# edmundhung/SparkFM

Measured on AMD Instinct MI355X. Metric: nnz_per_sec_fm_sgd_training, higher is better.
Workload: dtype f32

## Files before the change

### sparkfm_amd/csrc/fm_forward.hip

```cpp
#include "fm_device.h"

#ifndef FMHIP_FWD_LDS_SHARE
#define FMHIP_FWD_LDS_SHARE 1
#endif
#ifndef FMHIP_FWD_AHEAD
#define FMHIP_FWD_AHEAD 1
#endif
#ifndef FMHIP_FWD_W_SPLIT
#define FMHIP_FWD_W_SPLIT 1
#endif
#ifndef FMHIP_EXP_NO_STREAM
#define FMHIP_EXP_NO_STREAM 0
#endif
#ifndef FMHIP_EXP_NO_MATH
#define FMHIP_EXP_NO_MATH 0
#endif
#ifndef FMHIP_EXP_NO_W
#define FMHIP_EXP_NO_W 0
#endif
#ifndef FMHIP_EXP_NO_GATHER
#define FMHIP_EXP_NO_GATHER 0
#endif
#ifndef FMHIP_EXP_L1_GATHER
#define FMHIP_EXP_L1_GATHER 0
// ... 5 lines not shown
#define FMHIP_EXP_PHASE_PROBE 0
#endif
#define FMHIP_FWD_ABLATIONS ((FMHIP_EXP_NO_STREAM ? 1 : 0) | (FMHIP_EXP_NO_MATH ? 2 : 0) | (FMHIP_EXP_NO_W ? 4 : 0) | (FMHIP_EXP_NO_GATHER ? 8 : 0) | \
                             (FMHIP_EXP_L1_GATHER ? 16 : 0) | (FMHIP_EXP_NO_HOT ? 32 : 0) | (FMHIP_EXP_PHASE_PROBE ? 64 : 0))
#if FMHIP_FWD_ABLATIONS && !defined(FMHIP_ABLATION_BUILD)
#error "a result-changing FMHIP_EXP_* ablation is set without FMHIP_ABLATION_BUILD: timing-only variants are built by tools/build_variant.sh"
#endif

namespace fmhip {
int forward_ablations() { return FMHIP_FWD_ABLATIONS; }
}

namespace fmhip {

std::atomic<int> g_tune[kTuneCount] = {60, 1, 0, 0, 2, 1, 0, 1, 0, 1, 0, 1, 4};

int padded_factors(int k) {
    int kp = 32;
    while (kp < k) kp <<= 1;
    return kp;
}

int forward_wt_occupancy(int Kp);

int forward_blocks_wt(int Kp, int64_t n_rows, int occ_cap) {
    const int64_t need = forward_blocks(Kp, n_rows);
    int occ = forward_wt_occupancy(Kp);
    if (occ_cap > 0 && occ_cap < occ) occ = occ_cap;
    const int64_t cap = (int64_t)256 * occ;
    return (int)(need < cap ? need : cap);
// ... 159 lines not shown
                if (MASKED) {
                    float4 tv = f4mul(t[j][jj], __int_as_float(xi[j]));
                    if (!live) tv = f4zero();
                    f4add(q[jj], tv);
                    f4sqacc(s[jj], tv);
                } else if (FMHIP_EXP_NO_MATH) {
                    q[jj].x += t[j][jj].x * __int_as_float(xi[j]);
                } else {
                    acc_entry(q[jj], s[jj], t[j][jj], __int_as_float(xi[j]));
                }
            }
        }
    }
}

template <int LPN, int J, int MODE, bool PACKED>
__device__ __forceinline__ void row_finish(const FwdArgs &a, int r, int l, float4 (&q)[J], float4 (&s)[J], float lin, float w0,
                                           float &st1, float &st2, float &stbad, float &stl) {
    constexpr int KP = 4 * LPN * J;
    const int kl = PACKED ? (a.pack_k >> 2) & (LPN - 1) : 0, kj = PACKED ? (a.pack_k >> 2) / LPN : 0, kc = a.pack_k & 3;
    if (fwd_mode(MODE) == kFwdPartA) {
        float sp = 0.f, lp = lin;
#pragma unroll
        for (int jj = 0; jj < J; ++jj) {
            float4 sj = s[jj];
            if (PACKED && jj == kj && l == kl) f4set(sj, kc, 0.f);
            sp += (sj.x + sj.y) + (sj.z + sj.w);
        }
#pragma unroll
        for (int m = LPN >> 1; m >= 1; m >>= 1) { sp += __shfl_xor(sp, m, LPN); lp += __shfl_xor(lp, m, LPN); }
        float4 *pr = reinterpret_cast<float4 *>(a.P + (size_t)r * KP) + l;
#pragma unroll
        for (int jj = 0; jj < J; ++jj) pr[jj * LPN] = q[jj];
        if (l == 0) { a.part_sl[2 * (size_t)r] = sp; a.part_sl[2 * (size_t)r + 1] = lp; }
// ... 9 lines not shown
                if (l == kl) { f4set(q[jj], kc, 0.f); f4set(s[jj], kc, 0.f); }
            }
        lin_all = a.sw * __shfl(lk, kl, LPN);
    }
    float u = 0.f;
#pragma unroll
    for (int jj = 0; jj < J; ++jj) u += f4sqminus(q[jj], s[jj]);
    float tot = fmaf(0.5f * a.sv * a.sv, u, a.sw * lin);
    if (fwd_mode(MODE) == kFwdPartB && l == 0) tot += fmaf(-0.5f * a.sv * a.sv, a.part_sl[2 * (size_t)r], a.sw * a.part_sl[2 * (size_t)r + 1]);
#pragma unroll
    for (int m = LPN >> 1; m >= 1; m >>= 1) tot += __shfl_xor(tot, m, LPN);
    const float yhat = w0 + (tot + lin_all);
    constexpr bool logistic = (MODE & kFwdLogistic) != 0;
    float e, lrow = 0.f;
    if constexpr (logistic) {
        const bool t = a.y[a.row0 + r] > 0.f;
        const float z = expf(-fabsf(yhat)), inv = 1.f / (1.f + z);
        const bool pos = yhat >= 0.f;
        e = t ? -(pos ? z * inv : inv) : (pos ? inv : z * inv);
        if constexpr (fwd_mode(MODE) == kFwdResidual) lrow = fmaxf(t ? -yhat : yhat, 0.f) + log1pf(z);
    } else {
        e = yhat - a.y[a.row0 + r];
    }
    if (fwd_mode(MODE) == kFwdTrain || fwd_mode(MODE) == kFwdPartB) {
        float4 *pr = reinterpret_cast<float4 *>(a.P + (size_t)r * KP) + l;
        const float es = e * a.sv;
#pragma unroll
        for (int jj = 0; jj < J; ++jj) {
            float4 o = f4mul(q[jj], es);
            if (PACKED && jj == kj && l == kl) f4set(o, kc, e);
            if (!PACKED && kEInP && jj == 0 && l < 8) o = embed_bits4(o, __float_as_uint(e) >> (4 * l));
            p_store(pr + jj * LPN, o);
        }
    } else if (fwd_mode(MODE) == kFwdQ) {
        float4 *pr = reinterpret_cast<float4 *>(a.P + (size_t)r * KP) + l;
#pragma unroll
        for (int jj = 0; jj < J; ++jj) pr[jj * LPN] = f4mul(q[jj], a.sv);
// ... 48 lines not shown
    float *wt = lds + (size_t)T * KP;
    {
        const float4 *src = reinterpret_cast<const float4 *>(a.V);
        float4 *dst = reinterpret_cast<float4 *>(vt);
        const int n4 = T * (KP / 4);
        for (int i = threadIdx.x; i < n4; i += kLdsBlock) dst[i] = src[i];
        for (int i = threadIdx.x; i < T; i += kLdsBlock) wt[i] = a.w[i];
    }
    __syncthreads();
    const int l = threadIdx.x & (LPN - 1);
    const int slot = threadIdx.x / LPN;
    const float w0 = *a.w0;
    const __amdgpu_buffer_rsrc_t vr = make_rsrc(a.V, a.v_bytes);
    float st1 = 0.f, st2 = 0.f, stbad = 0.f, stl = 0.f;
    for (int ri = blockIdx.x * SLOTS + slot; ri < a.n_rows; ri += gridDim.x * SLOTS) {
        const int r = a.order ? a.order[ri] : ri;
        const int64_t p0 = a.row_ptr[a.row0 + r], p1 = a.row_ptr[a.row0 + r + 1];
        float4 q[J], s[J];
#pragma unroll
        for (int jj = 0; jj < J; ++jj) { q[jj] = f4zero(); s[jj] = f4zero(); }
        float lin = 0.f;
        for (int64_t base = p0; base < p1; base += LPN) {
            const int64_t p = base + l;
            int c = -1;
            float x = 0.f;
            if (p < p1) {
                c = stream_load(a.col + p);
                x = stream_load(a.val + p);
                const float wv = c < T ? wt[c] : a.w[c];
                lin = fmaf(wv, x, lin);
            }
#pragma unroll
// ... 14 lines not shown
                        tl[j][jj] = lp[jj * LPN];
                    }
                }
#pragma unroll
                for (int j = 0; j < CH; ++j) {
#pragma unroll
                    for (int jj = 0; jj < J; ++jj) {
                        const float4 t = hot[j] ? tl[j][jj] : tg[j][jj];
                        const float4 tv = f4mul(t, xs[j]);
                        f4add(q[jj], tv);
                        f4sqacc(s[jj], tv);
                    }
                }
            }
        }
        row_finish<LPN, J, MODE, false>(a, r, l, q, s, lin, w0, st1, st2, stbad, stl);
    }
    block_stats<kLdsBlock, MODE == (kFwdResidual | kFwdLogistic)>(a.bsum, st1, st2, stbad, stl);
}

template <bool WT, bool BUF>
__device__ __forceinline__ float w_lookup(const FwdArgs &a, __amdgpu_buffer_rsrc_t wr, const float *wt, int T, int c) {
    if (BUF && FMHIP_FWD_W_SPLIT) {
        const bool in_tile = WT && (uint32_t)c < (uint32_t)T;
        const float wg = buf_load1(wr, in_tile ? kOob : (uint32_t)c * 4u);
        if (!WT) return wg;
        const float wl = wt[in_tile ? c : 0];
        return in_tile ? wl : wg;
    }
    const int cc = c < 0 ? 0 : c;
    const float v = (WT && cc < T) ? wt[cc] : a.w[cc];
// ... 12 lines not shown
    const int T = WT ? a.wt_rows : 0;
    const __amdgpu_buffer_rsrc_t vr = make_rsrc(a.V, a.v_bytes);
    const __amdgpu_buffer_rsrc_t wr = make_rsrc(a.w, a.v_bytes / KPW);
    const int32_t *colb = a.col + a.nz0;
    const float *valb = a.val + a.nz0;
    float st1 = 0.f, st2 = 0.f, stbad = 0.f, stl = 0.f;
    if (BUF && FMHIP_FWD_AHEAD) {
#if FMHIP_EXP_PHASE_PROBE
        {
            const bool late = FMHIP_EXP_PHASE_PROBE >= 1000 ? (((blockIdx.x >> 3) ^ (blockIdx.x >> 8)) & 1) != 0 : __builtin_amdgcn_readfirstlane((int)(threadIdx.x >> 6)) >= 2;
            if (late)
                for (int i = 0; i < FMHIP_EXP_PHASE_PROBE % 1000; ++i) __builtin_amdgcn_s_sleep(1);
        }
#endif
        for (int ri = blockIdx.x * SLOTS + slot; ri < a.n_rows; ri += gridDim.x * SLOTS) {
            const int r = a.order ? a.order[ri] : ri;
            float4 xh = f4zero();
            if (HOT) xh = hot_load(a, r, l);
            const uint32_t p0 = (uint32_t)((fwd_mode(MODE) == kFwdPartB ? a.row_split[a.row0 + r] : a.row_ptr[a.row0 + r]) - a.nz0),
                           p1 = (uint32_t)((fwd_mode(MODE) == kFwdPartA ? a.row_split[a.row0 + r] : a.row_ptr[a.row0 + r + 1]) - a.nz0);
            float4 q[J], s[J];
#pragma unroll
            for (int jj = 0; jj < J; ++jj) {
                q[jj] = fwd_mode(MODE) == kFwdPartB ? reinterpret_cast<const float4 *>(a.P + (size_t)r * KPW)[jj * LPN + l] : f4zero();
                s[jj] = f4zero();
            }
            float lin = 0.f;
            if (HOT && !FMHIP_EXP_NO_HOT) {
                if (hot_plain) hot_prologue<LPN, J, !PACKED, false>(xh, vh, wh, l, q, s, lin);
                else hot_prologue<LPN, J, !PACKED, true>(xh, vh, wh, l, q, s, lin);
            }
            int c_n = -1;
            float x_n = 0.f;
            bool live_n = p0 + l < p1;
            if (live_n) { c_n = stream_load(colb + (p0 + l)); x_n = stream_load(valb + (p0 + l)); }
// ... 8 lines not shown
                    typedef __attribute__((address_space(1))) const float gflt;
                    gint *cp = (gint *)(live_n ? colb + pos : reinterpret_cast<const int32_t *>(a.w0));
                    gflt *xp = (gflt *)(live_n ? valb + pos : a.w0);
                    asm volatile("" : "+v"(cp), "+v"(xp));
                    c_n = *cp;
                    x_n = *xp;
                } else {
                    live_n = true; c_n = -1; x_n = 0.f;
                    if (pos < p1) { c_n = stream_load(colb + pos); x_n = stream_load(valb + pos); }
                }
                float wv = 0.f;
                if (!PACKED && !FMHIP_EXP_NO_W && c >= 0) wv = w_lookup<WT, BUF>(a, wr, wt, T, c);
                fwd_step<LPN, J, CH, false, BUF, PH == 1>(a.V, vr, slot_publish<LPN>(stage, c, x, l), c, x, LPN, l, q, s);
                if (!PACKED) lin = fmaf(wv, x, lin);
            }
            row_finish<LPN, J, MODE, PACKED>(a, r, l, q, s, lin, w0, st1, st2, stbad, stl);
        }
        block_stats<kBlock, MODE == (kFwdResidual | kFwdLogistic)>(a.bsum, st1, st2, stbad, stl);
        return;
    }
    for (int ri = blockIdx.x * SLOTS + slot; ri < a.n_rows; ri += gridDim.x * SLOTS) {
        const int r = a.order ? a.order[ri] : ri;
        float4 xh = f4zero();
        if (HOT) xh = hot_load(a, r, l);
        const uint32_t p0 = (uint32_t)((fwd_mode(MODE) == kFwdPartB ? a.row_split[a.row0 + r] : a.row_ptr[a.row0 + r]) - a.nz0),
                       p1 = (uint32_t)((fwd_mode(MODE) == kFwdPartA ? a.row_split[a.row0 + r] : a.row_ptr[a.row0 + r + 1]) - a.nz0);
        float4 q[J], s[J];
#pragma unroll
        for (int jj = 0; jj < J; ++jj) {
            q[jj] = fwd_mode(MODE) == kFwdPartB ? reinterpret_cast<const float4 *>(a.P + (size_t)r * KPW)[jj * LPN + l] : f4zero();
            s[jj] = f4zero();
        }
        float lin = 0.f;
        if (HOT && !FMHIP_EXP_NO_HOT) {
            if (hot_plain) hot_prologue<LPN, J, !PACKED, false>(xh, vh, wh, l, q, s, lin);
            else hot_prologue<LPN, J, !PACKED, true>(xh, vh, wh, l, q, s, lin);
        }
        uint32_t base = p0;
        for (; base + LPN <= p1; base += LPN) {
            const int c = FMHIP_EXP_NO_STREAM ? (int)((base + l) & 1023u) : stream_load(colb + (base + l));
            const float x = FMHIP_EXP_NO_STREAM ? 1.f : stream_load(valb + (base + l));
// ... 2 lines not shown
            fwd_step<LPN, J, CH, false, BUF>(a.V, vr, slot_publish<LPN>(stage, c, x, l), c, x, LPN, l, q, s);
            if (!PACKED) lin = fmaf(wv, x, lin);
        }
        if (base < p1) {
            const uint32_t p = base + l;
            int c = BUF ? -1 : 0;
            float x = 0.f, wv = 0.f;
            if (p < p1) {
                c = stream_load(colb + p);
                x = stream_load(valb + p);
                if (!PACKED && !FMHIP_EXP_NO_W) wv = w_lookup<WT, BUF>(a, wr, wt, T, c);
            }
            fwd_step<LPN, J, CH, !BUF, BUF>(a.V, vr, slot_publish<LPN>(stage, c, x, l), c, x, (int)(p1 - base), l, q, s);
            if (!PACKED) lin = fmaf(wv, x, lin);
        }
        row_finish<LPN, J, MODE, PACKED>(a, r, l, q, s, lin, w0, st1, st2, stbad, stl);
    }
    block_stats<kBlock, MODE == (kFwdResidual | kFwdLogistic)>(a.bsum, st1, st2, stbad, stl);
}

#ifndef FMHIP_FWD_PLAIN_WGS
#define FMHIP_FWD_PLAIN_WGS 5
#endif
template <int LPN, int J, int MODE, bool PACKED, bool HOT, bool BUF>
__global__ __launch_bounds__(kBlock, (LPN * J <= 8 && HOT ? FMHIP_FWD_PLAIN_WGS : 1)) void k_forward(FwdArgs a) {
    constexpr int KP = 4 * LPN * J;
    __shared__ __attribute__((aligned(16))) float vh[HOT ? kHotT * KP : 4];
    __shared__ float wh[HOT ? kHotT : 1];
    bool hot_plain = false;
    if (HOT) hot_plain = hot_stage<KP>(a, vh, wh);
    forward_rows<LPN, J, MODE, PACKED, HOT, false, BUF>(a, nullptr, vh, wh, hot_plain);
// ... 14 lines not shown
    else __syncthreads();
    forward_rows<LPN, J, MODE, false, HOT, true, BUF, PH>(a, wt, vh, wh, hot_plain);
}

template <int LPN, int J, int MODE, bool PACKED>
__global__ __launch_bounds__(kBlock) void k_forward_pass_b(FwdArgs a) {
    constexpr int KP = 4 * LPN * J;
    constexpr int SLOTS = kBlock / LPN;
    const int l = threadIdx.x & (LPN - 1);
    const int slot = threadIdx.x / LPN;
    const float w0 = *a.w0;
    const int32_t *colb = a.col + a.nz0;
    const float *valb = a.val + a.nz0;
    float st1 = 0.f, st2 = 0.f, stbad = 0.f, stl = 0.f;
    for (int ri = blockIdx.x * SLOTS + slot; ri < a.n_rows; ri += gridDim.x * SLOTS) {
        const int r = a.order ? a.order[ri] : ri;
        const uint32_t p0 = (uint32_t)(a.row_split[a.row0 + r] - a.nz0), p1 = (uint32_t)(a.row_ptr[a.row0 + r + 1] - a.nz0);
        float4 q[J], s[J];
#pragma unroll
        for (int jj = 0; jj < J; ++jj) {
            q[jj] = reinterpret_cast<const float4 *>(a.P + (size_t)r * KP)[jj * LPN + l];
            s[jj] = f4zero();
        }
        float lin = 0.f;
        for (uint32_t p = p0; p < p1; ++p) {
            const int c = colb[p];
            const float x = valb[p];
            const float4 *vp = reinterpret_cast<const float4 *>(a.V + (size_t)(uint32_t)c * KP) + l;
#pragma unroll
            for (int jj = 0; jj < J; ++jj) acc_entry(q[jj], s[jj], vp[jj * LPN], x);
            if (!PACKED && l == 0) lin = fmaf(a.w[c], x, lin);
        }
        row_finish<LPN, J, MODE, PACKED>(a, r, l, q, s, lin, w0, st1, st2, stbad, stl);
    }
    block_stats<kBlock, false>(a.bsum, st1, st2, stbad, stl);
}

__global__ __launch_bounds__(kBlock) void k_reduce_blocks(const double *bsum, int32_t nblocks, int32_t n_rows, float *scal,
                                                         double *acc) {
    __shared__ double sh[3][kBlock / 64];
    reduce_blocks_body(bsum, nblocks, n_rows, scal, acc, sh);
}

__global__ __launch_bounds__(kBlock) void k_reduce_blocks_logloss(const double *bsum, int32_t nblocks, int32_t n_rows, float *scal,
                                                                 double *acc) {
    __shared__ double sh[4][kBlock / 64];
    reduce_blocks_body<true>(bsum, nblocks, n_rows, scal, acc, sh);
}
// ... 80 lines not shown
hipError_t fwd_launch_pass(const FwdArgs &a0, hipStream_t s, int *n_partials) {
    if constexpr (LPN * J > 16) {
        return hipErrorInvalidValue;
    } else {
        FwdArgs a = a0;
        const bool hot_here = a.hot_T && (fwd_mode(MODE) == kFwdPartB) == (a.hot_in_b != 0);
        if (!hot_here) a.hot_T = 0;
        if (fwd_mode(MODE) == kFwdPartB) a.variant = 0;
        if (a.variant == 20) a.variant = a.hot_T ? 60 : 0;
        const FwdPlan pl = fwd_plan<LPN, J>(a);
        if (n_partials) *n_partials = pl.blocks;
        const dim3 g((unsigned)pl.blocks), b(kBlock);
        const bool buf = a.v_bytes != 0;
        if constexpr (fwd_mode(MODE) == kFwdPartB) {
            if (!a.hot_T) {
                a.order = nullptr;
                if (a.pack_k >= 0) hipLaunchKernelGGL((k_forward_pass_b<LPN, J, MODE, true>), g, b, 0, s, a);
                else hipLaunchKernelGGL((k_forward_pass_b<LPN, J, MODE, false>), g, b, 0, s, a);
                return hipGetLastError();
            }
        }
        if constexpr (fwd_mode(MODE) == kFwdPartA) {
            if (pl.var == 60) {
                const size_t lds_bytes = (size_t)a.wt_rows * sizeof(float);
                if (a.hot_T) {
                    if (buf) launch_wt<LPN, J, MODE, true, true>(a, g, b, lds_bytes, s);
                    else launch_wt<LPN, J, MODE, true, false>(a, g, b, lds_bytes, s);
                } else {
                    if (buf) launch_wt<LPN, J, MODE, false, true>(a, g, b, lds_bytes, s);
                    else launch_wt<LPN, J, MODE, false, false>(a, g, b, lds_bytes, s);
                }
// ... 110 lines not shown
```

### sparkfm_amd/csrc/fm_kernels.h

```cpp
#pragma once
#include <hip/hip_runtime.h>
#include <stdint.h>

#include <atomic>

#include "fm_constants.h"

namespace fmhip {

constexpr int kPartPad = 4;
constexpr int kScalars = 8;
constexpr int kGradHead = 32;

enum { kTuneFwd = 0, kTuneBwd = 1, kTuneTile = 2, kTuneRowBlock = 3, kTuneXcd = 4, kTuneHot = 5, kTuneFwdOcc = 6, kTuneRowOrder = 7,
       kTuneFlat = 8, kTuneLazy = 9, kTuneFused = 10, kTuneMerged = 11, kTuneHotPages = 12, kTuneCount = 13 };
constexpr int hot_pages_max(int Kp) { return Kp <= 32 ? 8 : (Kp <= 64 ? 4 : 1); }
extern std::atomic<int> g_tune[kTuneCount];
inline int tune_default(int key) { return g_tune[key].load(std::memory_order_relaxed); }

int padded_factors(int k);
constexpr int kMaxFwdBlocks = 16384;
int forward_blocks(int Kp, int64_t n_rows);
int forward_blocks_lds(int64_t n_rows);
int forward_blocks_wt(int Kp, int64_t n_rows, int occ_cap = 0);

enum FwdMode { kFwdTrain = 0, kFwdResidual = 1, kFwdQ = 2, kFwdPartA = 3, kFwdPartB = 4 };
enum Loss { kLossSquared = 0, kLossLogistic = 1 };
constexpr int kFwdLogistic = 8, kFwdModeMask = 7;
constexpr int fwd_mode(int mode) { return mode & kFwdModeMask; }

struct FwdArgs {
    const int64_t *row_ptr;
    const int32_t *col;
    const float *val;
    const float *y;
    const float *V;
    uint32_t v_bytes;
    const float *w;
    const float *w0;
    int64_t row0;
    int64_t nz0;
    const int64_t *row_split;
    float *part_sl;
    int32_t hot_in_b;
    const int32_t *order;
    int32_t n_rows;
    float *P;
    float *e;
    float *yhat;
    double *bsum;
    int32_t tile_rows;
    int32_t wt_rows;
    int32_t pack_k;
    int32_t hot_T;
    const float *xhot;
    const int32_t *hot_ids;
    float sv, sw;
    int32_t variant;
    int32_t occ_cap;
    int32_t phase;
    int32_t loss;
};

struct FusedUpd {
    float *V, *w;
    float sv, eta_v, eta_w, invb;
};

struct HotArgs {
    const float *P;
    const float *e;
    const float *xhot;
    int64_t page_stride;
    const int32_t *hot_ids;
    float *part;
    float *GV, *Gw, *Gb;
    int32_t n_rows;
// ... 97 lines not shown
```

### sparkfm_amd/csrc/fmhip_dataset.hip

```cpp
#include "fmhip_internal.h"
#include "../../include/fmhip_weights.h"
#include "csc_build.h"

#include <rocprim/device/device_radix_sort.hpp>

#include <algorithm>
#include <chrono>
#include <cstdio>
#include <memory>
#include <new>
#include <type_traits>
#include <vector>

using namespace fmhip;
using namespace fmhip::host;

static_assert(FMHIP_HOT_PAGES == kHotPages, "header and kernels disagree on the hot pages");
static_assert(FMHIP_RANGE_LEN == kRangeLen, "header and kernels disagree on the CSC range length");

namespace fmhip {
namespace host {


template <typename T>
// ... 236 lines not shown
        bm.split_short_off = append(split_short, hb.split_short, &bm.n_split_short);
        d.max_pieces = std::max(d.max_pieces, bm.n_pieces);
        d.max_ranges = std::max(d.max_ranges, bm.n_ranges);
        HostBatch().cfeat.swap(hb.cfeat);
    }
    d.h_cfeat = cfeat;
    d.h_cptr = cptr;
    d.h_split = split_seg;
    d.h_split_short = split_short;
    TRY(upload(d.cfeat, cfeat.data(), cfeat.size())); TRY(upload(d.cptr, cptr.data(), cptr.size()));
    TRY(upload(d.range_seg, range_seg.data(), range_seg.size()));
    TRY(upload(d.split_seg, split_seg.data(), split_seg.size())); TRY(upload(d.split_short, split_short.data(), split_short.size()));
    TRY(upload(d.cdst, cdst.data(), cdst.size()));
    TRY(upload(d.mp_feat, mp_feat.data(), mp_feat.size())); TRY(upload(d.mp_ptr, mp_ptr.data(), mp_ptr.size()));
    return upload(d.own_bits, own.data(), own.size());
}

template <typename FT>
int dataset_create_impl(int device, int64_t n_rows, const int64_t *row_ptr, const int32_t *col, const FT *val,
                        const FT *y, int64_t batch_rows, bool scoring, fmhip_dataset_t *out, int hot_opt = -1,
                        int64_t rb_opt = -1, const double *weight = nullptr) {
    const bool want_hot = hot_opt < 0 ? tune_default(kTuneHot) > 0 : hot_opt > 0;
    const int max_hot_pages = std::max(1, std::min(kHotPages, hot_opt > 0 ? hot_opt : tune_default(kTuneHotPages)));
    const int64_t want_rb = rb_opt < 0 ? std::max(tune_default(kTuneRowBlock), 0) : rb_opt;
    if (!out) return fail(FMHIP_ERR_INVALID, "out is NULL");
    *out = nullptr;
    if (n_rows < 0) return fail(FMHIP_ERR_INVALID, "n_rows < 0");
    if (!row_ptr) return fail(FMHIP_ERR_INVALID, "row_ptr is NULL");
    if (row_ptr[0] != 0) return fail(FMHIP_ERR_INVALID, "row_ptr[0] must be 0");
    PhaseTimer pt;
// ... 29 lines not shown
        if (hb.pages) {
            sp = split_hot_rows(n_rows, row_ptr, col, val, dim, batch_rows, hb, T);
            split = true;
            d->hot_T = kHotT;
            d->hot_pages = hb.pages;
            d->hot_ids.swap(hb.hot_ids);
            d->hot_max_id = *std::max_element(d->hot_ids.begin(), d->hot_ids.end());
            d->hot0_max_id = *std::max_element(d->hot_ids.begin(), d->hot_ids.begin() + kHotT);
        }
    }
    pt.lap("hot block: choose + split");
    const int64_t *sp_row_ptr = split ? sp.sp_ptr.data() : row_ptr;
    const int32_t *sp_col = split ? sp.sp_col.get() : col;
    TRY(batch_table(*d, sp_row_ptr, row_ptr, split ? &sp : nullptr));
    const int64_t nnz_s = d->nnz_sparse;
    {
        const char *ow = getenv("FMHIP_ORDER_WINDOW");
        const std::vector<int32_t> order = forward_row_order(n_rows, batch_rows, sp_row_ptr, ow ? atoll(ow) : 0, T);
        TRY(upload(d->row_order, order.data(), order.size()));
    }
    pt.lap("row order + upload");
    {
        std::vector<float> valf;
        const float *val_up = split ? sp.sp_val.get() : reinterpret_cast<const float *>(val);
        if (!split && !std::is_same<FT, float>::value) {
            valf = converted<float>(val, nnz_s, host_threads(nnz_s));
            val_up = valf.data();
        }
        const std::vector<float> yf = y ? converted<float>(y, n_rows, 1) : std::vector<float>((size_t)n_rows, 0.f);
        TRY(upload(d->row_ptr, sp_row_ptr, (size_t)n_rows + 1)); TRY(upload(d->col, sp_col, (size_t)nnz_s));
        TRY(upload(d->val, val_up, (size_t)nnz_s)); TRY(upload(d->y, yf.data(), (size_t)n_rows));
        if (weight) {
            const std::vector<float> cf = converted<float>(weight, n_rows, 1);
            for (float c : cf) d->weight_sum += (double)c;
            TRY(upload(d->c, cf.data(), (size_t)n_rows));
            d->weighted = true;
        }
        if (!scoring) { TRY(d->crow.alloc((size_t)nnz_s)); TRY(d->cval.alloc((size_t)nnz_s)); }
        if (split) {
            TRY(d->xhot.alloc((size_t)std::max<int64_t>(n_rows, 1) * kHotT * (size_t)d->hot_pages));
            TRY(upload(d->d_hot_ids, d->hot_ids.data(), d->hot_ids.size()));
            TRY(upload_hot_pages(*d, sp.xhot0.get()));
        }
    }
    sp.xhot0.reset();
    sp.sp_val.reset();
    pt.lap("fp32 re-pack + H2D");
    if (scoring) {
        *out = d.release();
        return FMHIP_OK;
    }
    const bool keep64 = !split && nb == 1 && nnz <= kAlsMaxNnz;
    if (keep64) TRY(upload_als_copies(*d, row_ptr, col, val, y, T));
    std::vector<HostBatch> hbs((size_t)nb);
    TRY(build_transposes(*d, keep64, want_rb, sp.drop_bits, hbs));
    pt.lap("device transposes + metadata");
    TRY(pack_column_index(*d, hbs));
    pt.lap("pack + upload column index");
    *out = d.release();
    return FMHIP_OK;
}

__global__ __launch_bounds__(256) void k_row_partition(const int64_t *row_ptr, int64_t n_rows, const int32_t *col, const float *val, int32_t cut,
                                                       int32_t *col_out, float *val_out, int64_t *split) {
    const int64_t r = (int64_t)blockIdx.x * 256 + threadIdx.x;
    if (r >= n_rows) return;
    const int64_t p0 = row_ptr[r], p1 = row_ptr[r + 1];
    int64_t h = p0;
    for (int64_t p = p0; p < p1; ++p)
        if (col[p] < cut) { col_out[h] = col[p]; val_out[h] = val[p]; ++h; }
    split[r] = h;
    for (int64_t p = p0; p < p1; ++p)
        if (col[p] >= cut) { col_out[h] = col[p]; val_out[h] = val[p]; ++h; }
// ... 377 lines not shown
```

### sparkfm_amd/csrc/fmhip_host.cpp

```cpp
#include "fmhip_host.h"
#include "mcmc_rng.h"

#include <stdlib.h>

#include <math.h>

#include <algorithm>
#include <atomic>
#include <cfloat>
#include <cmath>
#include <numeric>

namespace fmhip {
namespace host {

int host_threads(int64_t work_items) {
    unsigned hc = std::thread::hardware_concurrency();
    int64_t t = hc ? (int64_t)hc : 4;
    if (const char *e = getenv("FMHIP_HOST_THREADS")) t = atoi(e);
    t = std::min<int64_t>({t, 32, work_items / 65536 + 1});
    return (int)std::max<int64_t>(t, 1);
}

void shard_bounds(int64_t n_rows, const int64_t *row_ptr, int world, int rank, int64_t *lo, int64_t *hi) {
// ... 258 lines not shown
                for (int64_t r = w0; r < w1; ++r) maxlen = std::max(maxlen, row_ptr[row0 + r + 1] - row_ptr[row0 + r]);
                start.assign((size_t)maxlen + 2, 0);
                for (int64_t r = w0; r < w1; ++r) ++start[(size_t)(maxlen - (row_ptr[row0 + r + 1] - row_ptr[row0 + r])) + 1];
                for (size_t i = 1; i < start.size(); ++i) start[i] += start[i - 1];
                for (int64_t r = w0; r < w1; ++r) {
                    const size_t key = (size_t)(maxlen - (row_ptr[row0 + r + 1] - row_ptr[row0 + r]));
                    order[(size_t)(row0 + w0 + start[key]++)] = (int32_t)r;
                }
                if (window > 0 && ((w0 / win) & 1)) std::reverse(order.begin() + (row0 + w0), order.begin() + (row0 + w1));
            }
        }
    });
    return order;
}

template <typename FT>
SortedRows sort_rows_by_feature(int64_t n_rows, const int64_t *row_ptr, const int32_t *col, const FT *val, int threads) {
    SortedRows s;
    s.scol.resize((size_t)row_ptr[n_rows]);
    s.sval.resize((size_t)row_ptr[n_rows]);
    std::vector<char> dupv((size_t)threads, 0);
    parallel_chunks(n_rows, threads, [&](int t, int64_t lo, int64_t hi) {
        std::vector<int32_t> idx;
        bool dup = false;
        for (int64_t r = lo; r < hi; ++r) {
            const int64_t p0 = row_ptr[r], len = row_ptr[r + 1] - p0;
            idx.resize((size_t)len);
            std::iota(idx.begin(), idx.end(), 0);
            std::stable_sort(idx.begin(), idx.end(), [&](int32_t x, int32_t y) { return col[p0 + x] < col[p0 + y]; });
            for (int64_t j = 0; j < len; ++j) {
// ... 522 lines not shown
```

### sparkfm_amd/csrc/fmhip_host.h

```cpp
#pragma once
#include <stdint.h>

#include <memory>
#include <thread>
#include <vector>

#include "fm_constants.h"

namespace fmhip {
namespace host {

int host_threads(int64_t work_items);

template <class F>
void parallel_chunks(int64_t n, int threads, F f) {
    if (threads <= 1 || n <= 0) { f(0, (int64_t)0, n); return; }
    std::vector<std::thread> pool;
    pool.reserve((size_t)threads);
    for (int t = 0; t < threads; ++t) {
        const int64_t lo = n * t / threads, hi = n * (t + 1) / threads;
        pool.emplace_back([=]() { f(t, lo, hi); });
    }
    for (auto &th : pool) th.join();
}
// ... 18 lines not shown
constexpr int64_t kHotExactNnz = (int64_t)8 << 20;
struct HotBlock { int pages = 0; size_t p0 = 0; std::vector<int32_t> hot_ids; std::vector<int8_t> slot; std::vector<int64_t> kept; };
template <typename FT>
HotBlock choose_hot_block(int64_t n_rows, const int64_t *row_ptr, const int32_t *col, const FT *val, int32_t dim, int max_pages, bool row_blocked,
                          int threads, int64_t exact_nnz = kHotExactNnz);
struct HotSplit {
    std::vector<int64_t> sp_ptr, bwd_out;
    std::unique_ptr<int32_t[]> sp_col;
    std::unique_ptr<float[]> sp_val, xhot0;
    std::vector<slotmask_t> hot_masks; std::vector<uint32_t> drop_bits;
};
template <typename FT>
HotSplit split_hot_rows(int64_t n_rows, const int64_t *row_ptr, const int32_t *col, const FT *val, int32_t dim, int64_t batch_rows, HotBlock &hb,
                        int threads);
std::vector<int32_t> forward_row_order(int64_t n_rows, int64_t batch_rows, const int64_t *row_ptr, int64_t window, int threads);
struct SortedRows { std::vector<int32_t> scol; std::vector<double> sval; bool dup = false; };
template <typename FT>
SortedRows sort_rows_by_feature(int64_t n_rows, const int64_t *row_ptr, const int32_t *col, const FT *val, int threads);

struct HostBatch {
    std::vector<int32_t> cfeat, cptr, range_seg, split_seg, split_short, cdst, mp_feat, mp_ptr;
    int32_t n_feats = 0, n_pieces = 0;
};
void finish_batch_meta(HostBatch &hb, int32_t nnz, std::vector<int32_t> &cnt, std::vector<int32_t> &base);
std::vector<uint32_t> own_bitmaps(const std::vector<HostBatch> &hbs, const std::vector<int32_t> &hot_ids, int32_t dim);

enum { kWalkOrderStream = 0, kWalkOrderColdFirst = 1 };
constexpr int64_t kCostUnit = 20, kCloseCost = 53;
int64_t range_cost(const HostBatch &hb, int32_t cnnz, int32_t rho);
int walk_order_default();
// ... 90 lines not shown
```

### sparkfm_amd/csrc/fmhip_internal.h

```cpp
#pragma once
#include "../../include/fmhip_experimental.h"
#include "../../include/fmhip_pairing.h"
#include "../../include/fmhip_relational.h"
#include "../../include/fmhip_bpr.h"
#include "fm_kernels.h"
#include "fmhip_host.h"

#include <cmath>
#include <cstdarg>
#include <cstdint>
#include <cstring>
#include <memory>
#include <mutex>
#include <shared_mutex>
#include <string>
#include <vector>

namespace fmhip {
struct AlsArgs;
struct ColumnPlan;
namespace host {

int fail(int code, const char *fmt, ...) __attribute__((format(printf, 2, 3)));

// ... 157 lines not shown
    template <typename T> using DevBuf = fmhip::host::DevBuf<T>;
    int device = 0;
    int64_t n_rows = 0, nnz = 0, dimension = 0, batch_rows = 0;
    int64_t max_rows = 0;
    int32_t max_ranges = 0;
    std::vector<BatchMeta> batches;
    DevBuf<int64_t> row_ptr;
    DevBuf<int32_t> col;
    DevBuf<float> val, y;
    DevBuf<float> c;
    bool weighted = false;
    double weight_sum = 0.0;
    DevBuf<uint32_t> crow;
    DevBuf<float> cval;
    DevBuf<int32_t> row_order;
    DevBuf<int64_t> row_split;
    int64_t split_cut = -1;
    DevBuf<int32_t> col_part;
    DevBuf<float> val_part;
    std::mutex part_mu;
    int part_users = 0;
    int32_t hot0_max_id = -1;
    DevBuf<int32_t> cfeat, cptr, range_seg, split_seg, split_short, cdst, mp_feat, mp_ptr;
    DevBuf<uint32_t> own_bits;
    int64_t own_words = 0;
    DevBuf<int32_t> xlist;
    std::vector<int32_t> h_xlist;
    std::vector<int32_t> h_cfeat, h_cptr, h_split, h_split_short;
    int64_t rb_rows = 0;
    int32_t max_pieces = 0;
// ... 196 lines not shown
```

### sparkfm_amd/csrc/fmhip_step.hip

```cpp
#include "fmhip_internal.h"
#include "fm_pairing.h"
#include "fm_weights.h"

#include <algorithm>
#include <atomic>
#include <cassert>
#include <chrono>
#include <cmath>
#include <cstdarg>
#include <cstdio>
#include <cstring>
#include <memory>
#include <new>
#include <numeric>
#include <string>
#include <thread>
#include <type_traits>
#include <vector>

using namespace fmhip;

#ifndef FMHIP_FIN_BLOCKS
#define FMHIP_FIN_BLOCKS 2048
#endif
// ... 82 lines not shown
    a.row_ptr = d->row_ptr.p;
    a.col = d->col.p;
    a.val = d->val.p;
    a.y = d->y.p;
    a.V = m->V.p;
    {
        const uint64_t vb = (uint64_t)m->n1p * m->Kp * sizeof(float);
        a.v_bytes = (vb < 0xffffffffull && !m->tv(kTuneFlat)) ? (uint32_t)vb : 0u;
    }
    a.sv = (float)m->sv;
    a.sw = (float)m->sw;
    a.w = m->w.p;
    a.w0 = m->w0.p;
    a.row0 = bm.row0;
    a.nz0 = bm.nnz0;
    a.order = (m->tv(kTuneRowOrder) && (m->Kp >= 64 || getenv("FMHIP_ORDER_ALL"))) ? d->row_order.p + bm.row0 : nullptr;
    a.n_rows = (int32_t)bm.rows;
    a.P = m->P.p;
    a.e = m->e.p;
    a.yhat = nullptr;
    a.pack_k = m->pack_k();
    a.hot_T = d->hot_T;
    a.xhot = d->hot_T ? d->xhot.p + (size_t)bm.row0 * kHotT : nullptr;
    a.hot_ids = d->d_hot_ids.p;
    a.bsum = m->bsum.p;
    a.loss = m->rule.loss;
    {
        int64_t t = (128 * 1024) / ((int64_t)m->Kp * 4);
        if (m->tv(kTuneTile) > 0) t = m->tv(kTuneTile);
        a.tile_rows = (int32_t)std::min<int64_t>(t, m->n1);
        a.wt_rows = (int32_t)std::min<int64_t>(m->tv(kTuneTile) > 0 ? m->tv(kTuneTile) : 6144, m->n1);
// ... 461 lines not shown
```

Before: 43.70 billion.

## Permute CSR col/val into forward walk order so row streams are sequential

At dataset load, the nonzeros of each batch are reordered on the device so rows sit in the order the forward kernel visits them (row_order), and a permuted row_ptr, row_pos map and walk-ordered labels are uploaded. The forward kernels then index row_ptr and y by walk position and use the original row index only for the P and e outputs. The aim is contiguous streaming of col and val instead of jumping around the arrays, and it also turns on row ordering for small Kp. In exchange there is extra preprocessing and device memory, and every other consumer of row_ptr, col and val must agree with the permuted layout.

After: 44.09 billion, median of 6. Within noise of the previous version (+0.9%).

```diff
diff --git a/sparkfm_amd/csrc/fm_forward.hip b/sparkfm_amd/csrc/fm_forward.hip
--- a/sparkfm_amd/csrc/fm_forward.hip
+++ b/sparkfm_amd/csrc/fm_forward.hip
@@ -43,6 +43,12 @@
 namespace fmhip {
 
 std::atomic<int> g_tune[kTuneCount] = {60, 1, 0, 0, 2, 1, 0, 1, 0, 1, 0, 1, 4};
+
+void walk_in_caller_order(FwdArgs &a) {
+    const bool walk_stream = a.walk != kWalkNone;
+    a.order = walk_stream ? a.pos : nullptr;
+    a.walk = walk_stream ? kWalkPos : kWalkNone;
+}
 
 int padded_factors(int k) {
     int kp = 32;
@@ -232,10 +238,16 @@
     }
 }
 
+__device__ __forceinline__ int walk_lookup(const FwdArgs &a, int ri) { return a.order ? a.order[ri] : ri; }
+__device__ __forceinline__ int walk_row(const FwdArgs &a, int ri, int x) { return a.walk == kWalkPos ? ri : x; }
+__device__ __forceinline__ int walk_pos(const FwdArgs &a, int ri, int x) { return a.walk == kWalkOrder ? ri : x; }
+
 template <int LPN, int J, int MODE, bool PACKED>
-__device__ __forceinline__ void row_finish(const FwdArgs &a, int r, int l, float4 (&q)[J], float4 (&s)[J], float lin, float w0,
+__device__ __forceinline__ void row_finish(const FwdArgs &a, int ri, int x, int l, float4 (&q)[J], float4 (&s)[J], float lin, float w0,
                                            float &st1, float &st2, float &stbad, float &stl) {
     constexpr int KP = 4 * LPN * J;
+    asm volatile("" : "+v"(x));
+    const int r = walk_row(a, ri, x);
     const int kl = PACKED ? (a.pack_k >> 2) & (LPN - 1) : 0, kj = PACKED ? (a.pack_k >> 2) / LPN : 0, kc = a.pack_k & 3;
     if (fwd_mode(MODE) == kFwdPartA) {
         float sp = 0.f, lp = lin;
@@ -275,13 +287,13 @@
     constexpr bool logistic = (MODE & kFwdLogistic) != 0;
     float e, lrow = 0.f;
     if constexpr (logistic) {
-        const bool t = a.y[a.row0 + r] > 0.f;
+        const bool t = a.y[a.row0 + walk_pos(a, ri, x)] > 0.f;
         const float z = expf(-fabsf(yhat)), inv = 1.f / (1.f + z);
         const bool pos = yhat >= 0.f;
         e = t ? -(pos ? z * inv : inv) : (pos ? inv : z * inv);
         if constexpr (fwd_mode(MODE) == kFwdResidual) lrow = fmaxf(t ? -yhat : yhat, 0.f) + log1pf(z);
     } else {
-        e = yhat - a.y[a.row0 + r];
+        e = yhat - a.y[a.row0 + walk_pos(a, ri, x)];
     }
     if (fwd_mode(MODE) == kFwdTrain || fwd_mode(MODE) == kFwdPartB) {
         float4 *pr = reinterpret_cast<float4 *>(a.P + (size_t)r * KP) + l;
@@ -360,8 +372,9 @@
     const __amdgpu_buffer_rsrc_t vr = make_rsrc(a.V, a.v_bytes);
     float st1 = 0.f, st2 = 0.f, stbad = 0.f, stl = 0.f;
     for (int ri = blockIdx.x * SLOTS + slot; ri < a.n_rows; ri += gridDim.x * SLOTS) {
-        const int r = a.order ? a.order[ri] : ri;
-        const int64_t p0 = a.row_ptr[a.row0 + r], p1 = a.row_ptr[a.row0 + r + 1];
+        const int x = walk_lookup(a, ri);
+        const int wi = walk_pos(a, ri, x);
+        const int64_t p0 = a.row_ptr[a.row0 + wi], p1 = a.row_ptr[a.row0 + wi + 1];
         float4 q[J], s[J];
 #pragma unroll
         for (int jj = 0; jj < J; ++jj) { q[jj] = f4zero(); s[jj] = f4zero(); }
@@ -406,7 +419,7 @@
                 }
             }
         }
-        row_finish<LPN, J, MODE, false>(a, r, l, q, s, lin, w0, st1, st2, stbad, stl);
+        row_finish<LPN, J, MODE, false>(a, ri, x, l, q, s, lin, w0, st1, st2, stbad, stl);
     }
     block_stats<kLdsBlock, MODE == (kFwdResidual | kFwdLogistic)>(a.bsum, st1, st2, stbad, stl);
 }
@@ -449,11 +462,12 @@
         }
 #endif
         for (int ri = blockIdx.x * SLOTS + slot; ri < a.n_rows; ri += gridDim.x * SLOTS) {
-            const int r = a.order ? a.order[ri] : ri;
+            const int x = walk_lookup(a, ri);
+            const int r = walk_row(a, ri, x), wi = walk_pos(a, ri, x);
             float4 xh = f4zero();
             if (HOT) xh = hot_load(a, r, l);
-            const uint32_t p0 = (uint32_t)((fwd_mode(MODE) == kFwdPartB ? a.row_split[a.row0 + r] : a.row_ptr[a.row0 + r]) - a.nz0),
-                           p1 = (uint32_t)((fwd_mode(MODE) == kFwdPartA ? a.row_split[a.row0 + r] : a.row_ptr[a.row0 + r + 1]) - a.nz0);
+            const uint32_t p0 = (uint32_t)((fwd_mode(MODE) == kFwdPartB ? a.row_split[a.row0 + wi] : a.row_ptr[a.row0 + wi]) - a.nz0),
+                           p1 = (uint32_t)((fwd_mode(MODE) == kFwdPartA ? a.row_split[a.row0 + wi] : a.row_ptr[a.row0 + wi + 1]) - a.nz0);
             float4 q[J], s[J];
 #pragma unroll
             for (int jj = 0; jj < J; ++jj) {
@@ -492,17 +506,18 @@
                 fwd_step<LPN, J, CH, false, BUF, PH == 1>(a.V, vr, slot_publish<LPN>(stage, c, x, l), c, x, LPN, l, q, s);
                 if (!PACKED) lin = fmaf(wv, x, lin);
             }
-            row_finish<LPN, J, MODE, PACKED>(a, r, l, q, s, lin, w0, st1, st2, stbad, stl);
+            row_finish<LPN, J, MODE, PACKED>(a, ri, x, l, q, s, lin, w0, st1, st2, stbad, stl);
         }
         block_stats<kBlock, MODE == (kFwdResidual | kFwdLogistic)>(a.bsum, st1, st2, stbad, stl);
         return;
     }
     for (int ri = blockIdx.x * SLOTS + slot; ri < a.n_rows; ri += gridDim.x * SLOTS) {
-        const int r = a.order ? a.order[ri] : ri;
+        const int x = walk_lookup(a, ri);
+        const int r = walk_row(a, ri, x), wi = walk_pos(a, ri, x);
         float4 xh = f4zero();
         if (HOT) xh = hot_load(a, r, l);
-        const uint32_t p0 = (uint32_t)((fwd_mode(MODE) == kFwdPartB ? a.row_split[a.row0 + r] : a.row_ptr[a.row0 + r]) - a.nz0),
-                       p1 = (uint32_t)((fwd_mode(MODE) == kFwdPartA ? a.row_split[a.row0 + r] : a.row_ptr[a.row0 + r + 1]) - a.nz0);
+        const uint32_t p0 = (uint32_t)((fwd_mode(MODE) == kFwdPartB ? a.row_split[a.row0 + wi] : a.row_ptr[a.row0 + wi]) - a.nz0),
+                       p1 = (uint32_t)((fwd_mode(MODE) == kFwdPartA ? a.row_split[a.row0 + wi] : a.row_ptr[a.row0 + wi + 1]) - a.nz0);
         float4 q[J], s[J];
 #pragma unroll
         for (int jj = 0; jj < J; ++jj) {
@@ -535,7 +550,7 @@
             fwd_step<LPN, J, CH, !BUF, BUF>(a.V, vr, slot_publish<LPN>(stage, c, x, l), c, x, (int)(p1 - base), l, q, s);
             if (!PACKED) lin = fmaf(wv, x, lin);
         }
-        row_finish<LPN, J, MODE, PACKED>(a, r, l, q, s, lin, w0, st1, st2, stbad, stl);
+        row_finish<LPN, J, MODE, PACKED>(a, ri, x, l, q, s, lin, w0, st1, st2, stbad, stl);
     }
     block_stats<kBlock, MODE == (kFwdResidual | kFwdLogistic)>(a.bsum, st1, st2, stbad, stl);
 }
@@ -580,8 +595,9 @@
     const float *valb = a.val + a.nz0;
     float st1 = 0.f, st2 = 0.f, stbad = 0.f, stl = 0.f;
     for (int ri = blockIdx.x * SLOTS + slot; ri < a.n_rows; ri += gridDim.x * SLOTS) {
-        const int r = a.order ? a.order[ri] : ri;
-        const uint32_t p0 = (uint32_t)(a.row_split[a.row0 + r] - a.nz0), p1 = (uint32_t)(a.row_ptr[a.row0 + r + 1] - a.nz0);
+        const int x = walk_lookup(a, ri);
+        const int r = walk_row(a, ri, x), wi = walk_pos(a, ri, x);
+        const uint32_t p0 = (uint32_t)(a.row_split[a.row0 + wi] - a.nz0), p1 = (uint32_t)(a.row_ptr[a.row0 + wi + 1] - a.nz0);
         float4 q[J], s[J];
 #pragma unroll
         for (int jj = 0; jj < J; ++jj) {
@@ -597,7 +613,7 @@
             for (int jj = 0; jj < J; ++jj) acc_entry(q[jj], s[jj], vp[jj * LPN], x);
             if (!PACKED && l == 0) lin = fmaf(a.w[c], x, lin);
         }
-        row_finish<LPN, J, MODE, PACKED>(a, r, l, q, s, lin, w0, st1, st2, stbad, stl);
+        row_finish<LPN, J, MODE, PACKED>(a, ri, x, l, q, s, lin, w0, st1, st2, stbad, stl);
     }
     block_stats<kBlock, false>(a.bsum, st1, st2, stbad, stl);
 }
@@ -708,7 +724,7 @@
         const bool buf = a.v_bytes != 0;
         if constexpr (fwd_mode(MODE) == kFwdPartB) {
             if (!a.hot_T) {
-                a.order = nullptr;
+                walk_in_caller_order(a);
                 if (a.pack_k >= 0) hipLaunchKernelGGL((k_forward_pass_b<LPN, J, MODE, true>), g, b, 0, s, a);
                 else hipLaunchKernelGGL((k_forward_pass_b<LPN, J, MODE, false>), g, b, 0, s, a);
                 return hipGetLastError();
diff --git a/sparkfm_amd/csrc/fm_kernels.h b/sparkfm_amd/csrc/fm_kernels.h
--- a/sparkfm_amd/csrc/fm_kernels.h
+++ b/sparkfm_amd/csrc/fm_kernels.h
@@ -29,6 +29,8 @@
 constexpr int kFwdLogistic = 8, kFwdModeMask = 7;
 constexpr int fwd_mode(int mode) { return mode & kFwdModeMask; }
 
+enum { kWalkNone = 0, kWalkOrder = 1, kWalkPos = 2 };
+
 struct FwdArgs {
     const int64_t *row_ptr;
     const int32_t *col;
@@ -44,6 +46,8 @@
     float *part_sl;
     int32_t hot_in_b;
     const int32_t *order;
+    const int32_t *pos;
+    int32_t walk;
     int32_t n_rows;
     float *P;
     float *e;
@@ -61,6 +65,8 @@
     int32_t phase;
     int32_t loss;
 };
+
+void walk_in_caller_order(FwdArgs &a);
 
 struct FusedUpd {
     float *V, *w;
diff --git a/sparkfm_amd/csrc/fmhip_dataset.hip b/sparkfm_amd/csrc/fmhip_dataset.hip
--- a/sparkfm_amd/csrc/fmhip_dataset.hip
+++ b/sparkfm_amd/csrc/fmhip_dataset.hip
@@ -274,6 +274,49 @@
     TRY(upload(d.cdst, cdst.data(), cdst.size()));
     TRY(upload(d.mp_feat, mp_feat.data(), mp_feat.size())); TRY(upload(d.mp_ptr, mp_ptr.data(), mp_ptr.size()));
     return upload(d.own_bits, own.data(), own.size());
+}
+
+__global__ __launch_bounds__(256) void k_walk_gather(const int64_t *row_ptr, const int64_t *walk_ptr, const int32_t *order, int64_t row0, int64_t rows,
+                                                     const int32_t *col, const float *val, int32_t *col_out, float *val_out) {
+    const int64_t i = ((int64_t)blockIdx.x * 256 + threadIdx.x) >> 3;
+    const int l = threadIdx.x & 7;
+    if (i >= rows) return;
+    const int64_t r = row0 + order[row0 + i];
+    const int64_t src = row_ptr[r], len = row_ptr[r + 1] - src, dst = walk_ptr[row0 + i] - row_ptr[row0];
+    for (int64_t j = l; j < len; j += 8) { col_out[dst + j] = col[src + j]; val_out[dst + j] = val[src + j]; }
+}
+
+int walk_order_stream(fmhip_dataset &d, const int64_t *row_ptr, const std::vector<int32_t> &order, const std::vector<float> &y, int threads) {
+    const WalkLayout wl = walk_layout(d.n_rows, d.batch_rows, row_ptr, order.data(), threads);
+    std::vector<float> yw((size_t)d.n_rows);
+    parallel_chunks(d.n_rows, threads, [&](int, int64_t lo, int64_t hi) {
+        for (int64_t g = lo; g < hi; ++g) {
+            const int64_t row0 = g / d.batch_rows * d.batch_rows;
+            yw[(size_t)g] = y[(size_t)(row0 + order[(size_t)g])];
+        }
+    });
+    TRY(upload(d.row_pos, wl.row_pos.data(), wl.row_pos.size()));
+    TRY(upload(d.y_walk, yw.data(), yw.size()));
+    DevBuf<int64_t> wp;
+    TRY(upload(wp, wl.walk_ptr.data(), wl.walk_ptr.size()));
+    int32_t max_nnz = 0;
+    for (const BatchMeta &bm : d.batches) max_nnz = std::max(max_nnz, bm.nnz);
+    DevBuf<int32_t> stage;
+    TRY(stage.alloc(2 * (size_t)max_nnz));
+    for (const BatchMeta &bm : d.batches) {
+        if (bm.nnz == 0) continue;
+        int32_t *sc = stage.p;
+        float *sv = reinterpret_cast<float *>(stage.p + max_nnz);
+        hipLaunchKernelGGL(k_walk_gather, dim3((unsigned)((bm.rows * 8 + 255) / 256)), dim3(256), 0, nullptr, d.row_ptr.p, wp.p, d.row_order.p, bm.row0, bm.rows,
+                           d.col.p, d.val.p, sc, sv);
+        HIP_TRY(hipGetLastError());
+        HIP_TRY(hipMemcpyAsync(d.col.p + bm.nnz0, sc, (size_t)bm.nnz * sizeof(int32_t), hipMemcpyDeviceToDevice, nullptr));
+        HIP_TRY(hipMemcpyAsync(d.val.p + bm.nnz0, sv, (size_t)bm.nnz * sizeof(float), hipMemcpyDeviceToDevice, nullptr));
+    }
+    HIP_TRY(hipMemcpyAsync(d.row_ptr.p, wp.p, wl.walk_ptr.size() * sizeof(int64_t), hipMemcpyDeviceToDevice, nullptr));
+    HIP_TRY(hipStreamSynchronize(nullptr));
+    d.walk_stream = true;
+    return FMHIP_OK;
 }
 
 template <typename FT>
@@ -333,12 +376,17 @@
     const int32_t *sp_col = split ? sp.sp_col.get() : col;
     TRY(batch_table(*d, sp_row_ptr, row_ptr, split ? &sp : nullptr));
     const int64_t nnz_s = d->nnz_sparse;
+    std::vector<int32_t> order;
     {
         const char *ow = getenv("FMHIP_ORDER_WINDOW");
-        const std::vector<int32_t> order = forward_row_order(n_rows, batch_rows, sp_row_ptr, ow ? atoll(ow) : 0, T);
+        order = forward_row_order(n_rows, batch_rows, sp_row_ptr, ow ? atoll(ow) : 0, T);
         TRY(upload(d->row_order, order.data(), order.size()));
     }
     pt.lap("row order + upload");
+    const bool keep64 = !scoring && !split && nb == 1 && nnz <= kAlsMaxNnz;
+    const char *ws = getenv("FMHIP_WALK_STREAM");
+    const bool walk = n_rows > 0 && !keep64 && !(ws && atoi(ws) == 0);
+    std::vector<float> yf;
     {
         std::vector<float> valf;
         const float *val_up = split ? sp.sp_val.get() : reinterpret_cast<const float *>(val);
@@ -346,7 +394,7 @@
             valf = converted<float>(val, nnz_s, host_threads(nnz_s));
             val_up = valf.data();
         }
-        const std::vector<float> yf = y ? converted<float>(y, n_rows, 1) : std::vector<float>((size_t)n_rows, 0.f);
+        yf = y ? converted<float>(y, n_rows, 1) : std::vector<float>((size_t)n_rows, 0.f);
         TRY(upload(d->row_ptr, sp_row_ptr, (size_t)n_rows + 1)); TRY(upload(d->col, sp_col, (size_t)nnz_s));
         TRY(upload(d->val, val_up, (size_t)nnz_s)); TRY(upload(d->y, yf.data(), (size_t)n_rows));
         if (weight) {
@@ -366,16 +414,19 @@
     sp.sp_val.reset();
     pt.lap("fp32 re-pack + H2D");
     if (scoring) {
+        if (walk) TRY(walk_order_stream(*d, sp_row_ptr, order, yf, T));
+        pt.lap("stream into walk order");
         *out = d.release();
         return FMHIP_OK;
     }
-    const bool keep64 = !split && nb == 1 && nnz <= kAlsMaxNnz;
     if (keep64) TRY(upload_als_copies(*d, row_ptr, col, val, y, T));
     std::vector<HostBatch> hbs((size_t)nb);
     TRY(build_transposes(*d, keep64, want_rb, sp.drop_bits, hbs));
     pt.lap("device transposes + metadata");
     TRY(pack_column_index(*d, hbs));
     pt.lap("pack + upload column index");
+    if (walk) TRY(walk_order_stream(*d, sp_row_ptr, order, yf, T));
+    pt.lap("stream into walk order");
     *out = d.release();
     return FMHIP_OK;
 }
diff --git a/sparkfm_amd/csrc/fmhip_host.cpp b/sparkfm_amd/csrc/fmhip_host.cpp
--- a/sparkfm_amd/csrc/fmhip_host.cpp
+++ b/sparkfm_amd/csrc/fmhip_host.cpp
@@ -296,6 +296,27 @@
     return order;
 }
 
+WalkLayout walk_layout(int64_t n_rows, int64_t batch_rows, const int64_t *row_ptr, const int32_t *order, int threads) {
+    WalkLayout w;
+    w.row_pos.resize((size_t)n_rows);
+    w.walk_ptr.resize((size_t)n_rows + 1);
+    w.walk_ptr[(size_t)n_rows] = row_ptr[n_rows];
+    const int64_t nb = n_rows > 0 ? (n_rows + batch_rows - 1) / batch_rows : 0;
+    parallel_chunks(nb, std::min<int>(threads, (int)std::max<int64_t>(nb, 1)), [&](int, int64_t blo, int64_t bhi) {
+        for (int64_t b = blo; b < bhi; ++b) {
+            const int64_t row0 = b * batch_rows, rows = std::min(batch_rows, n_rows - row0);
+            int64_t at = row_ptr[row0];
+            for (int64_t i = 0; i < rows; ++i) {
+                const int64_t r = order[row0 + i];
+                w.row_pos[(size_t)(row0 + r)] = (int32_t)i;
+                w.walk_ptr[(size_t)(row0 + i)] = at;
+                at += row_ptr[row0 + r + 1] - row_ptr[row0 + r];
+            }
+        }
+    });
+    return w;
+}
+
 template <typename FT>
 SortedRows sort_rows_by_feature(int64_t n_rows, const int64_t *row_ptr, const int32_t *col, const FT *val, int threads) {
     SortedRows s;
diff --git a/sparkfm_amd/csrc/fmhip_host.h b/sparkfm_amd/csrc/fmhip_host.h
--- a/sparkfm_amd/csrc/fmhip_host.h
+++ b/sparkfm_amd/csrc/fmhip_host.h
@@ -56,6 +56,8 @@
 HotSplit split_hot_rows(int64_t n_rows, const int64_t *row_ptr, const int32_t *col, const FT *val, int32_t dim, int64_t batch_rows, HotBlock &hb,
                         int threads);
 std::vector<int32_t> forward_row_order(int64_t n_rows, int64_t batch_rows, const int64_t *row_ptr, int64_t window, int threads);
+struct WalkLayout { std::vector<int32_t> row_pos; std::vector<int64_t> walk_ptr; };
+WalkLayout walk_layout(int64_t n_rows, int64_t batch_rows, const int64_t *row_ptr, const int32_t *order, int threads);
 struct SortedRows { std::vector<int32_t> scol; std::vector<double> sval; bool dup = false; };
 template <typename FT>
 SortedRows sort_rows_by_feature(int64_t n_rows, const int64_t *row_ptr, const int32_t *col, const FT *val, int threads);
diff --git a/sparkfm_amd/csrc/fmhip_internal.h b/sparkfm_amd/csrc/fmhip_internal.h
--- a/sparkfm_amd/csrc/fmhip_internal.h
+++ b/sparkfm_amd/csrc/fmhip_internal.h
@@ -195,6 +195,9 @@
     DevBuf<uint32_t> crow;
     DevBuf<float> cval;
     DevBuf<int32_t> row_order;
+    bool walk_stream = false;
+    DevBuf<int32_t> row_pos;
+    DevBuf<float> y_walk;
     DevBuf<int64_t> row_split;
     int64_t split_cut = -1;
     DevBuf<int32_t> col_part;
diff --git a/sparkfm_amd/csrc/fmhip_step.hip b/sparkfm_amd/csrc/fmhip_step.hip
--- a/sparkfm_amd/csrc/fmhip_step.hip
+++ b/sparkfm_amd/csrc/fmhip_step.hip
@@ -120,7 +120,13 @@
     a.w0 = m->w0.p;
     a.row0 = bm.row0;
     a.nz0 = bm.nnz0;
-    a.order = (m->tv(kTuneRowOrder) && (m->Kp >= 64 || getenv("FMHIP_ORDER_ALL"))) ? d->row_order.p + bm.row0 : nullptr;
+    a.order = (m->tv(kTuneRowOrder) && (m->Kp >= 64 || d->walk_stream || getenv("FMHIP_ORDER_ALL"))) ? d->row_order.p + bm.row0 : nullptr;
+    if (d->walk_stream) {
+        a.walk = kWalkOrder;
+        a.pos = d->row_pos.p + bm.row0;
+        a.y = d->y_walk.p;
+        if (!a.order) walk_in_caller_order(a);
+    }
     a.n_rows = (int32_t)bm.rows;
     a.P = m->P.p;
     a.e = m->e.p;
```
